# Gadersd/stable-diffusion-xl-burn

Hardware: AMD Instinct MI355X
Metric: images/sec SDXL-base 1024x1024 30-step CFG7.5 (whole job); UNet step ms p50 (higher is better)
Workload: dtype f16; 1 GPU; SDXL-base 1024x1024, n_steps=30 (31 CFG UNet step pairs), CFG 7.5, batch 1 prompt/GPU + VAE decode to u8 (BASELINE configs[1]); precision=f16, vae_dtype=f32_split, weights=synthetic seeded (random-init SDXL-base architecture), mix_classes=0, parallelism=replica x1, 1 prompt per GPU, weights broadcast once over RCCL, hipgraph=True, split_cfg=False, fused_xattn=True, pipelined_decode=False, prompts_per_call=1, full=False, library=stable-diffusion-xl-burn_amd/lib/libsdxl_mi355.so, debug_set=

## Files before the change

stable-diffusion-xl-burn_amd/build.py:

```python
from __future__ import annotations

import hashlib
import os
import subprocess
import sys
from concurrent.futures import ThreadPoolExecutor

HERE = os.path.dirname(os.path.abspath(__file__))
CSRC = os.path.join(HERE, "csrc")
OBJ = os.path.join(HERE, "build")
LIBDIR = os.path.join(HERE, "lib")
LIB = os.path.join(LIBDIR, "libsdxl_mi355.so")
ARCH = "gfx950"
SOURCES = ["igemm.hip", "igemm_glds.hip", "igemm_wreg.hip", "igemm_measure.hip", "norm.hip", "attention.hip", "elementwise.hip", "capi.hip", "capi_ops.hip",
           "select.cpp", "specs.cpp", "weights.cpp", "unet.cpp", "vae.cpp", "sampler.cpp", "clip.cpp", "comm.cpp"]
FLAGS = ["-O3", "-std=c++17", "-fPIC", f"--offload-arch={ARCH}", "-Wall", "-Wno-unused-function",
         "-Wno-unused-result"]


def _hipcc() -> str:
    for c in (os.environ.get("HIPCC"), "/opt/rocm/bin/hipcc", "hipcc"):
        if c and (os.path.isabs(c) and os.path.exists(c) or not os.path.isabs(c)):
            return c
    raise RuntimeError("hipcc not found")


def _measure() -> bool:
    return os.environ.get("SDXL_MEASURE") == "1"

# ... 57 lines not shown
```

stable-diffusion-xl-burn_amd/csrc/capi.hip:

```cpp
#include "capi_internal.h"
#include "select_debug.h"
#include <algorithm>
#include <cstring>

using namespace sdxl;

thread_local std::string sdxl::g_err;

namespace {
template <class H, class F> void create_handle(sdxl_ctx* ctx, H** out, F make) {
  std::unique_ptr<H> h(new H());
  h->ctx = ctx;
  make(*h);
  *out = h.release();
}
UNetCfg to_cfg(const sdxl_unet_config* c) {
  SDXL_REQUIRE(c != nullptr, "null config");
  SDXL_REQUIRE(c->n_levels >= 1 && c->n_levels <= 8, "n_levels out of range");
  UNetCfg u;
  u.adm_in_channels = c->adm_in_channels; u.in_channels = c->in_channels; u.out_channels = c->out_channels;
  u.model_channels = c->model_channels; u.n_head_channels = c->n_head_channels; u.context_dim = c->context_dim;
  u.is_refiner = c->is_refiner != 0;
  for (int i = 0; i < c->n_levels; ++i) { u.channel_mults.push_back(c->channel_mults[i]); u.transformer_depths.push_back(c->transformer_depths[i]); }
  SDXL_REQUIRE(u.model_channels > 0 && u.n_head_channels > 0 && u.context_dim > 0 && u.adm_in_channels > 0, "bad UNet config");
// ... 101 lines not shown
  igemm_glds_init();
  *out = c;
  API_END
}
int sdxl_debug_set(const char* key, int value) {
  API_BEGIN
  SDXL_REQUIRE(key != nullptr, "null key");
  if (select_knob_set(key, value)) return SDXL_OK;
  else if (std::strcmp(key, "igemm_epilogue_staged") == 0) igemm_set_epilogue_staged(value);
  else if (std::strcmp(key, "hl_weights_exact") == 0) igemm_set_hl_weights_exact(value);
  else if (std::strcmp(key, "igemm_warm") == 0) igemm_set_warm(value);
  else if (std::strcmp(key, "splitk_wt") == 0) igemm_set_splitk_wt(value);
  else if (std::strcmp(key, "hl_demote") == 0) unet_set_hl_demote(value);
  else if (std::strcmp(key, "mix_classes") == 0) unet_set_mix_classes(value);
  else if (std::strcmp(key, "wreg_xcd2d") == 0) igemm_set_wreg_xcd2d(value);
#ifdef SDXL_MEASURE
  else if (std::strcmp(key, "xa_vec64") == 0) igemm_set_xa_vec64(value);
  else if (std::strcmp(key, "no_cfg") == 0) g_debug_no_cfg = value != 0;
#endif
  else throw Error(std::string("unknown debug key ") + key);
  API_END
}
int sdxl_debug_warm_schedule(int n, const unsigned* bytes, const unsigned char* host, int* warmed_by) {
  API_BEGIN
  WarmSeq ws;
  for (int j = 0; j < n; ++j)
    ws.seq.push_back(WarmSeq::Item{reinterpret_cast<const void*>((uintptr_t)(j + 1) << 12), bytes[j], host[j] != 0, host[j] ? 14u << 20 : 0u, {nullptr, nullptr, nullptr}, {0u, 0u, 0u}});
  ws.finish();
  for (int j = 0; j < n; ++j) warmed_by[j] = -1;
  for (int i = 0; i < n; ++i)
// ... 569 lines not shown
```

stable-diffusion-xl-burn_amd/csrc/elementwise.hip:

```cpp
#include "kernels.h"
#include <algorithm>
#include <stdexcept>

namespace sdxl {

typedef _Float16 half_t;
typedef _Float16 half8 __attribute__((ext_vector_type(8)));
typedef float f32x4 __attribute__((ext_vector_type(4)));

__device__ __forceinline__ float ld_f(const void* p, size_t i, int dt) {
  if (dt == DT_HL) { const half_t* b = reinterpret_cast<const half_t*>(p) + ((i >> 4) << 5) + (i & 15); return (float)b[0] + (float)b[16]; }
  return dt == DT_F16 ? (float)reinterpret_cast<const half_t*>(p)[i] : reinterpret_cast<const float*>(p)[i];
}
__device__ __forceinline__ void st_f(void* p, size_t i, int dt, float v) {
  if (dt == DT_HL) {
    half_t* b = reinterpret_cast<half_t*>(p) + ((i >> 4) << 5) + (i & 15);
    const half_t hi = (half_t)v;
    b[0] = hi; b[16] = (half_t)(v - (float)hi);
  } else if (dt == DT_F16) reinterpret_cast<half_t*>(p)[i] = (half_t)v; else reinterpret_cast<float*>(p)[i] = v;
}
__device__ __forceinline__ float silu_f(float x) { return x / (1.0f + expf(-x)); }

template <typename WT>
__global__ __launch_bounds__(256) void gemv_kernel(const GemvParams p, int cols) {
// ... 39 lines not shown
            const f32x4 xv = *reinterpret_cast<const f32x4*>(xr + j);
            acc[b] += xv[0] * wv[j] + xv[1] * wv[j + 1] + xv[2] * wv[j + 2] + xv[3] * wv[j + 3];
          }
        }
      }
    }
#pragma unroll
    for (int b = 0; b < 8; ++b) {
#pragma unroll
      for (int o = 32; o > 0; o >>= 1) acc[b] += __shfl_xor(acc[b], o);
    }
    if (lane == 0) {
      for (int b = 0; b < p.Bm; ++b) {
        float v = acc[b] + (p.bias ? p.bias[n] : 0.f);
        if (p.silu_out) v = silu_f(v);
        if (p.Yadd) v += p.Yadd[(size_t)b * p.ldy + n];
        p.Y[(size_t)b * p.ldy + n] = v;
      }
    }
  }
}
void launch_gemv(const GemvParams& pin, hipStream_t s) {
  const int ce = pin.w_dt == DT_F16 ? 8 : 4;
  const int Kx = (pin.K + 64 * ce - 1) / (64 * ce) * (64 * ce);
  const size_t row_bytes = (size_t)Kx * sizeof(float);
  if (row_bytes > 64 * 1024) throw std::runtime_error("gemv: K does not fit the 64 KiB input staging buffer");
  const int rows_per_launch = (int)std::min<size_t>(8, (64 * 1024) / row_bytes);
  for (int b0 = 0; b0 < pin.Bm; b0 += rows_per_launch) {
    GemvParams p = pin;
    p.Bm = std::min(rows_per_launch, pin.Bm - b0);
    p.X = pin.X + (size_t)b0 * pin.ldx;
    p.Y = pin.Y + (size_t)b0 * pin.ldy;
    if (pin.Yadd) p.Yadd = pin.Yadd + (size_t)b0 * pin.ldy;
    const size_t lds = (size_t)p.Bm * row_bytes;
    const int cols = p.N >= 8192 ? 4 : 1;
    dim3 g((p.N + 4 * cols - 1) / (4 * cols));
    if (p.w_dt == DT_F16) hipLaunchKernelGGL(gemv_kernel<half_t>, g, dim3(256), lds, s, p, cols);
    else hipLaunchKernelGGL(gemv_kernel<float>, g, dim3(256), lds, s, p, cols);
  }
}

__global__ __launch_bounds__(256) void softmax_rows_kernel(const float* S, int lds_, void* P, int p_dt, int ldp, int n,
                                                           int npad, float scale, const float* mask, int ldmask,
                                                           int mask_rows, float p_scale, float* p_scale_out) {
  __shared__ float red[8];
  const int row = blockIdx.x, tid = threadIdx.x;
  const float* s = S + (size_t)row * lds_;
  const float* mk = mask ? mask + (size_t)(row % mask_rows) * ldmask : nullptr;
// ... 428 lines not shown
  float z[4];
  seeded_normal4(seeds.v[b], (uint32_t)hw, draw, z);
#pragma unroll
  for (int c = 0; c < 4; ++c) out[((size_t)b * 4 + c) * HW + hw] = z[c];
}
void launch_seeded_noise(float* out, const uint64_t* seeds, uint32_t draw, int n, int HW, hipStream_t s) {
  for (int b0 = 0; b0 < n; b0 += kMaxSeeds) {
    const int nb = std::min(kMaxSeeds, n - b0);
    DdimSeeds k{};
    for (int b = 0; b < nb; ++b) k.v[b] = seeds[b0 + b];
    const size_t total = (size_t)nb * HW;
    hipLaunchKernelGGL(seeded_noise_kernel, dim3((total + 255) / 256), dim3(256), 0, s, out + (size_t)b0 * 4 * HW, k, draw, nb, HW);
  }
}

template <bool SEEDED>
__global__ void ddim_kernel(const DdimParams p, int do_update) {
#pragma clang fp contract(off)
  const size_t i = (size_t)blockIdx.x * blockDim.x + threadIdx.x;
  if (i >= (size_t)p.n * p.HW) return;
  const int b = i / p.HW;
  const int hw = i - (size_t)b * p.HW;
  const int idx = *p.step_idx;
  const int next = do_update ? idx + 1 : 0;
  float x[4];
#pragma unroll
  for (int c = 0; c < 4; ++c) x[c] = p.latent[((size_t)b * 4 + c) * p.HW + hw];
  if (do_update) {
    const StepCoef k = p.table[idx];
#pragma unroll
    for (int c = 0; c < 4; ++c) {
      const float ec = ld_f(p.eps, ((size_t)b * p.HW + hw) * p.eps_ld + c, p.eps_dt);
      float e = ec;
      if (p.use_cfg) {
// ... 25 lines not shown
        if constexpr (SEEDED) zn = z[c]; else zn = p.step_noise[(size_t)next * p.n * 4 * p.HW + e];
        x[c] = p.ref[e] * kn.sqrt_a + zn * kn.sqrt_1ma;
      }
    }
  }
#pragma unroll
  for (int c = 0; c < 4; ++c) p.latent[((size_t)b * 4 + c) * p.HW + hw] = x[c];
  for (int r = 0; r < p.in_rep; ++r)
#pragma unroll
    for (int c = 0; c < 4; ++c) st_f(p.unet_in, ((size_t)(r * p.n + b) * p.HW + hw) * p.in_ld + c, p.in_dt, x[c]);
}
template <bool SEEDED>
__global__ void dpmpp2m_kernel(const DdimParams p, int do_update) {
#pragma clang fp contract(off)
  const size_t i = (size_t)blockIdx.x * blockDim.x + threadIdx.x;
  if (i >= (size_t)p.n * p.HW) return;
  const int b = i / p.HW;
  const int hw = i - (size_t)b * p.HW;
  const int idx = *p.step_idx;
  const int next = do_update ? idx + 1 : 0;
  float x[4];
#pragma unroll
  for (int c = 0; c < 4; ++c) x[c] = p.latent[((size_t)b * 4 + c) * p.HW + hw];
  if (do_update) {
    const StepCoef k = p.table[idx];
    float x0p[4] = {0.f, 0.f, 0.f, 0.f};
    if (k.c_1 != 0.f) {
#pragma unroll
      for (int c = 0; c < 4; ++c) x0p[c] = p.hist[((size_t)b * 4 + c) * p.HW + hw];
    }
// ... 223 lines not shown
```

stable-diffusion-xl-burn_amd/csrc/engine.h:

```cpp
#pragma once
#include "kernels.h"

#include <map>
#include <memory>
#include <stdexcept>
#include <string>
#include <utility>
#include <vector>

namespace sdxl {

struct Error : std::runtime_error {
  explicit Error(const std::string& m) : std::runtime_error(m) {}
};
#define SDXL_HIP(x)                                                                                   \
  do {                                                                                                \
    hipError_t e__ = (x);                                                                             \
    if (e__ != hipSuccess) throw ::sdxl::Error(std::string(#x) + " failed: " + hipGetErrorString(e__)); \
  } while (0)
#define SDXL_REQUIRE(cond, msg)                          \
  do {                                                   \
    if (!(cond)) throw ::sdxl::Error(std::string(msg));  \
  } while (0)

// ... 259 lines not shown
void alloc_ln_operands(Exec& ex, const StPlan& pl, size_t M, int C, const Act& ln, LnOperands& o);
void want_ln_shadow(LnOperands& o, Epi& e, bool sh, LinForm f, const NormW& n);
struct LnIn { const Lin* w; Act a; const float* stat; };
LnIn ln_input(Exec& ex, LnOperands& o, const Lin& plain, const Lin& sh, LinForm f, const NormW& n, const Act& t, int cls);
constexpr size_t kGegluDirectRows = 256;
inline bool geglu_widened(LinForm f, const LnIn& in, size_t M) { return M < kGegluDirectRows && (in.stat || reads_f16(f)); }
struct BlockW { BlockDesc d; ResBlockW res; STW st; Lin conv; };

class UNet {
 public:
  UNet(const UNetCfg& cfg, int compute_dt, int stream_dt, WeightSource& src, hipStream_t st, int mix = 0);
  ~UNet();
  const UNetCfg& cfg() const { return cfg_; }
  void set_context(const float* context, int n_ctx, const float* label, int B, hipStream_t s);
  void forward(int B, int H, int W, const float* t_dev, int t_stride, hipStream_t s);
  void forward_nchw(const float* x, const int* timesteps, const float* context, int n_ctx, const float* label,
                    int B, int H, int W, float* out, hipStream_t s);
  void* unet_in(int B, int H, int W);
  float* eps_out() { return eps_; }
  int compute_dt() const { return cdt_; }
  int mix_classes() const { return mix_; }
  int input_dt() const { return cdt_ == DT_HL ? DT_F32 : cdt_; }
  int attn_dt() const { return cdt_ == DT_HL ? DT_F32 : cdt_; }
  void set_use_graph(bool g) { use_graph_ = g; }
  void set_split_cfg(bool on, int release_offset) { split_cfg_ = on; split_offset_ = release_offset; }
  void set_fused_cross_attention(bool on) { fuse_xattn_ = on; }
  void set_gn_from_producer(bool on) { gn_from_producer_ = on; }
  void profile(int B, int H, int W, float ms[Profiler::NCLS], int launches[Profiler::NCLS], double flops[Profiler::NCLS],
               hipStream_t s);
  float eager_ms(int B, int H, int W, hipStream_t s);
// ... 12 lines not shown
  int mix_ = 0;
  bool mix_knob_ = false;
  bool attn16_ = false;
  DeviceArena warena_;
  std::vector<BlockW> inp_, out_;
  BlockW mid_res1_, mid_res2_;
  Lin lin1_t_, lin2_t_, lin1_l_, lin2_l_, embcat_;
  NormW norm_out_; Lin conv_out_;
  int emb_total_ = 0;
  struct KV { void* k = nullptr; void* vt = nullptr; void* xa = nullptr; void* xa_lo = nullptr; };
  std::vector<std::vector<KV>> kv_;
  std::vector<const STW*> st_list_;
  DeviceArena ctx_arena_;
  int ctx_B_ = 0, n_ctx_ = 0, vt_ld_ctx_ = 0;
  float* label_emb_ = nullptr;
  int pB_ = 0, pH_ = 0, pW_ = 0;
  DeviceArena act_;
  void* in_ = nullptr; float* eps_ = nullptr;
  float *temb_ = nullptr, *g1_ = nullptr, *emb_ = nullptr, *ebias_ = nullptr, *gn_partial_ = nullptr, *tconv_ = nullptr;
  float* skws_[2] = {nullptr, nullptr}; unsigned* skcnt_[2] = {nullptr, nullptr}; size_t skws_bytes_ = 0;
  bool fuse_ln_ = false;
  bool use_graph_ = true;
  bool split_cfg_ = false; int split_offset_ = 0;
  bool plan_split_ = false; int graph_off_ = 0;
  bool fuse_xattn_ = true, plan_xattn_ = true;
  WarmSeq warm_;
  float* attn_xws_[2] = {nullptr, nullptr}; unsigned* attn_xcnt_[2] = {nullptr, nullptr};
  bool graph_warm_ = false;
  size_t attn_xcnt_bytes_ = 0;
  int demote_mask_ = 0, graph_demote_ = 0;
// ... 100 lines not shown
  void sample_latent_inpaint(const Conditioning& c, double cfg_scale, int n_steps, const float* reference,
                             const unsigned char* mask, const float* noise0, const float* step_noise, float* out,
                             hipStream_t s);
  void refine_latent(const float* latent, const Conditioning& c, double cfg_scale, int step_start, int n_steps,
                     const float* noise, float* out, hipStream_t s);
  void sample_latent_seeded(const Conditioning& c, double cfg_scale, int n_steps, const uint64_t* seeds, double eta, float* out,
                            hipStream_t s);
  void sample_latent_inpaint_seeded(const Conditioning& c, double cfg_scale, int n_steps, const float* reference,
                                    const unsigned char* mask, const uint64_t* seeds, double eta, float* out, hipStream_t s);
  void refine_latent_seeded(const float* latent, const Conditioning& c, double cfg_scale, int step_start, int n_steps,
                            const uint64_t* seeds, double eta, float* out, hipStream_t s);
  static std::vector<int> step_schedule(int n_steps, int step_start, int n_train);
  static void solver_coefficients(const double* alphas, int n_train, int n_steps, int step_start, int solver, double eta, double* out);
  void set_solver(int solver);
  int solver() const { return solver_; }
  std::vector<float> step_ms;
  bool time_steps = false;
  float* trace = nullptr; int trace_cap = 0;

 private:
  void ensure_state(size_t elems);
  void diffuse(float* latent, const Conditioning& c, int step_start, int n_steps, double cfg_scale, const float* reference,
               const unsigned char* mask, const float* step_noise, hipStream_t s, const uint64_t* seeds = nullptr, double eta = 0.0);
  std::unique_ptr<UNet> unet_;
  std::vector<double> alphas_;
  int n_train_;
  bool is_refiner_;
  float* latent_ = nullptr; size_t latent_cap_ = 0;
  float* noise_ = nullptr; size_t noise_cap_ = 0;
  float* hist_ = nullptr; size_t hist_cap_ = 0;
// ... 10 lines not shown
```

stable-diffusion-xl-burn_amd/csrc/kernels.h:

```cpp
#pragma once
#include <hip/hip_runtime.h>
#include <stdint.h>
#include <stdexcept>

namespace sdxl {

enum DType : int { DT_F32 = 0, DT_F16 = 1, DT_HL = 2 };

static inline size_t dt_size(int dt) { return dt == DT_F16 ? 2 : 4; }

struct IgemmParams {
  const void* A;
  const void* W;
  const void* Wf;
  int a_dt;
  int B, Hin, Win, Cin, lda;
  int Hout, Wout;
  int ksize, stride, pad, up;
  int M, N, K, Kpad;
  const float* bias;
  const float* ebias;
  int ebias_ld;
  int rpb;
  int act;
// ... 46 lines not shown
  int grid, block, lds;
};
IgemmChoice igemm_select(const IgemmParams& p, int compute_dt, const SelectKnobs& k);
bool igemm_gn_part_ok(const IgemmParams& p, const SelectKnobs& k);
bool igemm_wreg_selected(const IgemmParams& p, const SelectKnobs& k);
bool igemm_wreg_xattn_selected(const IgemmParams& p, const SelectKnobs& k);
bool igemm_xattn_ok(int a_dt, int c_dt, int M, int N, int K, int rpb, int n_ctx);
size_t xattn_pack_bytes(int B, int C);
void launch_xattn_pack(const void* K, const void* Vt, void* out, int B, int C, int n_ctx, int vt_ld, hipStream_t s);
int igemm_splitk_slices(const IgemmParams& p);
size_t igemm_splitk_ws_bytes(int batch, int rows_per_entry, int n_max);
constexpr int kSplitkCounters = 4096;
SelectKnobs igemm_launch_knobs();
void launch_igemm(const IgemmParams& p, int compute_dt, const SelectKnobs& knobs, hipStream_t s);
void launch_igemm(const IgemmParams& p, int compute_dt, hipStream_t s);
void launch_repack_wfrag(const void* w, void* wf, int Npad, int Kpad, hipStream_t s);
void igemm_set_warm(int v);
int igemm_warm_enabled();
void igemm_set_splitk_wt(int v);
void igemm_set_wreg_xcd2d(int v);
void igemm_set_hl_weights_exact(int v);
void igemm_set_xa_vec64(int v);
void igemm_set_epilogue_staged(int v);
#ifdef SDXL_MEASURE
void igemm_set_timeline(void* device_buf);
void igemm_set_wreg_timeline(void* device_buf);
void igemm_set_wide_timeline(void* device_buf);
int igemm_timeline_words();
#endif
constexpr int kMaxDevices = 64;
// ... 71 lines not shown
void attention_set_timeline(void* device_buf);
#endif

void launch_softmax_rows(const float* S, int lds, void* P, int p_dt, int ldp, int rows, int n, int npad, float scale,
                         const float* mask, int ldmask, int mask_rows, hipStream_t s, float p_scale = 1.0f, float* p_scale_out = nullptr);

struct GemvParams {
  const float* X; int ldx;
  const void* W; int w_dt; int Kpad;
  const float* bias;
  float* Y; int ldy;
  const float* Yadd;
  int Bm, N, K;
  int silu_in;
  int silu_out;
};
void launch_gemv(const GemvParams& p, hipStream_t s);

void launch_timestep_embedding(const float* t_dev, int t_stride, float* out, int Bm, int dim, hipStream_t s);
void launch_nchw_to_nhwc(const float* src, int src_batch_stride, void* dst, int dt, int B, int C, int HW, int ldd,
                         float scale, hipStream_t s);
void launch_nhwc_to_nchw(const void* src, int dt, int lds, float* dst, int B, int C, int HW, float scale, hipStream_t s);
void launch_copy_rows(const void* src, int sdt, int lds, void* dst, int ddt, int ldd, int rows, int C, hipStream_t s);
void launch_fill_zero(void* p, size_t bytes, hipStream_t s);
void launch_f16_exact(const float* src, size_t n, float wscale, float* exact, hipStream_t s, bool accumulate = false);
void launch_f32_to_hl(const void* src, int lds, void* dst, int ldd, size_t rows, int C, hipStream_t s);
void launch_f32_to_hl_scaled(const void* src, int lds, void* dst, int ldd, size_t rows, int C, float* scale_io, hipStream_t s, int nb = 1,
                             bool have_partials = false);
unsigned count_nonfinite(const void* src, int dt, int lds, size_t rows, int C, hipStream_t s);
void launch_f16_to_hl(const void* src, int lds, void* dst, int ldd, size_t rows, int C, hipStream_t s);
// ... 22 lines not shown
constexpr uint32_t kDrawInitial = 0;
constexpr uint32_t draw_blend(uint32_t i) { return 1u + 2u * i; }
constexpr uint32_t draw_sigma(uint32_t i) { return 2u + 2u * i; }
constexpr int kMaxSeeds = 8;
struct DdimSeeds { uint64_t v[kMaxSeeds]; };
struct DdimParams {
  float* latent;
  const void* eps; int eps_dt; int eps_ld;
  const StepCoef* table; int* step_idx;
  int n, HW; int use_cfg;
  const float* ref; const unsigned char* mask; const float* step_noise; int n_steps_total;
  int seeded; DdimSeeds seeds;
  void* unet_in; int in_dt; int in_ld; int in_rep;
  float* t_out;
  int solver; float* hist;
};
void launch_ddim_step(const DdimParams& p, int do_update, hipStream_t s);
void launch_seeded_noise(float* out, const uint64_t* seeds, uint32_t draw, int n, int HW, hipStream_t s);
void launch_axpby(float* dst, const float* a, float sa, const float* b, float sb, size_t n, hipStream_t s);
void launch_to_u8_image(const void* src, int dt, int lds, unsigned char* dst, size_t pixels, hipStream_t s);
void launch_from_u8_image(const unsigned char* src, void* dst, int dt, int ldd, size_t pixels, hipStream_t s);

void launch_synth_fill(float* dst, size_t numel, uint64_t key, float scale, float mean, hipStream_t s);
void launch_pack_linear(const float* src, void* dst, int dt, int K, int N, int Kpad, int Npad, int geglu,
                        int n_offset, hipStream_t s, const float* kscale = nullptr,
                        float wscale = 1.0f);
void launch_pack_linear_hilo(const float* src, void* dst, int K, int N, int Npad, int geglu, float lo_scale, hipStream_t s, int mode = 0, int n_offset = 0);
void launch_colsum_packed(const void* wp, int dt, int Kpad, int nrows, float* cs, hipStream_t s, const float* kscale = nullptr, int K = 0, int interleave = 0);
void launch_beta_dot(const float* w, const float* beta, const float* bias, float* out, int K, int N, hipStream_t s);
void launch_pack_conv(const float* src, void* dst, int dt, int Cout, int Cin, int ks, int Kpad, int Npad,
// ... 6 lines not shown
```

stable-diffusion-xl-burn_amd/csrc/sampler.cpp:

```cpp
#include "engine.h"

#include <algorithm>
#include <cmath>

namespace sdxl {

std::vector<int> Diffuser::step_schedule(int n_steps, int step_start, int n_train) {
  SDXL_REQUIRE(n_steps >= 1 && n_steps <= n_train, "n_steps out of range");
  const int step = n_train / n_steps;
  std::vector<int> ts;
  for (int t = n_train - step_start - 1; t >= 0; t -= step) ts.push_back(t);
  return ts;
}

Diffuser::Diffuser(const UNetCfg& cfg, int compute_dt, int stream_dt, WeightSource& src, const float* alphas_host,
                   int n_train, hipStream_t st, int mix)
    : n_train_(n_train), is_refiner_(cfg.is_refiner) {
  unet_.reset(new UNet(cfg, compute_dt, stream_dt, src, st, mix));
  alphas_.resize(n_train);
  for (int i = 0; i < n_train; ++i) alphas_[i] = (double)alphas_host[i];
  SDXL_HIP(hipMalloc((void**)&step_idx_, sizeof(int)));
  SDXL_HIP(hipMalloc((void**)&t_dev_, 8 * sizeof(float)));
}
Diffuser::~Diffuser() {
// ... 41 lines not shown
    const double A = -std::expm1(-(1.0 + eta) * h);
    c[0] = (sigma_p / sigma) * std::exp(-eta * h);
    c[3] = sigma_p * std::sqrt(-std::expm1(-2.0 * eta * h));
    if (have_prev) {
      const double r = h_prev / h;
      c[1] = alpha_p * A * (1.0 + 1.0 / (2.0 * r));
      c[2] = -alpha_p * A / (2.0 * r);
    } else {
      c[1] = alpha_p * A;
      c[2] = 0.0;
    }
    h_prev = h;
    have_prev = true;
  }
}

#ifdef SDXL_MEASURE
bool g_debug_no_cfg = false;
#else
static constexpr bool g_debug_no_cfg = false;
#endif

void Diffuser::diffuse(float* latent, const Conditioning& c, int step_start, int n_steps, double cfg_scale,
                       const float* reference, const unsigned char* mask, const float* step_noise, hipStream_t s,
                       const uint64_t* seeds, double eta) {
  UNet& u = *unet_;
  const UNetCfg& uc = u.cfg();
  const bool single = is_refiner_ || g_debug_no_cfg;
  const int n = c.n, B = single ? n : 2 * n;
  SDXL_REQUIRE(n >= 1 && B <= 8, "batch out of range");
// ... 51 lines not shown
      double sqrt_ap, sqrt_1map, sigma;
      ddim_terms(a, ap, eta, sqrt_ap, sqrt_1map, sigma);
      k.sqrt_ap = (float)sqrt_ap;
      k.sqrt_1map = (float)sqrt_1map;
      k.sigma = (float)sigma;
    }
    tab[i] = k;
  }
  tab[iters] = StepCoef{};
  if (iters + 1 > table_cap_) {
    if (table_) SDXL_HIP(hipFree(table_));
    SDXL_HIP(hipMalloc((void**)&table_, (size_t)(iters + 1) * sizeof(StepCoef)));
    table_cap_ = iters + 1;
  }
  SDXL_HIP(hipMemcpyAsync(table_, tab.data(), (size_t)(iters + 1) * sizeof(StepCoef), hipMemcpyHostToDevice, s));
  SDXL_HIP(hipStreamSynchronize(s));

  DdimParams p{};
  p.latent = latent;
  p.eps = u.eps_out(); p.eps_dt = DT_F32; p.eps_ld = uc.out_channels;
  p.table = table_; p.step_idx = step_idx_;
  p.n = n; p.HW = HW; p.use_cfg = single ? 0 : 1;
  p.ref = reference; p.mask = mask; p.step_noise = step_noise; p.n_steps_total = iters;
  p.unet_in = unet_in; p.in_dt = u.input_dt(); p.in_ld = uc.in_channels; p.in_rep = single ? 1 : 2;
  p.t_out = t_dev_;
  p.solver = solver_; p.hist = hist_;
  if (seeds) {
    p.seeded = 1;
    for (int b = 0; b < n; ++b) p.seeds.v[b] = seeds[b];
  }
  launch_ddim_step(p, 0, s);

  std::vector<hipEvent_t> ev;
  if (time_steps) {
    ev.resize(iters + 1);
    for (auto& e : ev) SDXL_HIP(hipEventCreate(&e));
    SDXL_HIP(hipEventRecord(ev[0], s));
  }
  for (int i = 0; i < iters; ++i) {
    u.forward(B, h, w, t_dev_, 0, s);
    launch_ddim_step(p, 1, s);
    if (trace && i < trace_cap)
      SDXL_HIP(hipMemcpyAsync(trace + (size_t)i * n * 4 * HW, latent, (size_t)n * 4 * HW * sizeof(float), hipMemcpyDeviceToDevice, s));
    if (time_steps) SDXL_HIP(hipEventRecord(ev[i + 1], s));
  }
  if (time_steps) {
    SDXL_HIP(hipEventSynchronize(ev[iters]));
    step_ms.assign(iters, 0.f);
    for (int i = 0; i < iters; ++i) SDXL_HIP(hipEventElapsedTime(&step_ms[i], ev[i], ev[i + 1]));
    for (auto& e : ev) (void)hipEventDestroy(e);
  }
}

static void ensure_latent(float*& buf, size_t& cap, size_t elems) {
  if (elems > cap) {
// ... 82 lines not shown
```

stable-diffusion-xl-burn_amd/csrc/unet.cpp:

```cpp
#include "engine.h"

#include <atomic>
#include <cmath>
#include <cstring>

namespace sdxl {

namespace {
ResBlockW load_res(WeightBuilder& wb, const std::string& p, int cin, int cout, std::vector<std::string>& emb_names,
                   int& emb_off) {
  ResBlockW r;
  r.cin = cin; r.cout = cout;
  r.norm_in = wb.norm(p + ".norm_in");
  r.conv_in = wb.conv(p + ".conv_in");
  r.norm_out = wb.norm(p + ".norm_out");
  r.conv_out = wb.conv(p + ".conv_out");
  r.has_skip = wb.has(p + ".skip_connection.weight");
  if (r.has_skip) r.skip = wb.conv(p + ".skip_connection");
  r.emb_off = emb_off;
  emb_names.push_back(p + ".lin_embed");
  emb_off += cout;
  return r;
}
const std::vector<std::string> kQkv = {".attn1.query", ".attn1.key", ".attn1.value"};
// ... 73 lines not shown
    t.qkv = pack_proj(wb, plan.qkv, qkv, false, plan.qkv_sh ? &t.qkv_sh : nullptr, q + ".norm1");
    t.out1 = pack_proj(wb, plan.out1, {q + kOut1}, false);
    t.n2 = wb.norm(q + ".norm2");
    t.q2 = pack_proj(wb, plan.q2, {q + kQ2}, false, plan.q2_sh ? &t.q2_sh : nullptr, q + ".norm2");
    t.kv2 = wb.fused_linear({q + ".attn2.key", q + ".attn2.value"});
    t.out2 = pack_proj(wb, plan.out2, {q + kOut2}, false);
    t.n3 = wb.norm(q + ".norm3");
    t.geglu = pack_proj(wb, plan.geglu, {q + kGeglu}, true, plan.geglu_sh ? &t.geglu_sh : nullptr, q + ".norm3");
    t.ff = pack_proj(wb, plan.ff, {q + kFf}, false);
    s.blocks.push_back(t);
  }
  s.proj_out = wb.linear(p + ".proj_out");
  return s;
}
void gemv(Exec& ex, const Lin& w, const float* x, int ldx, float* y, int ldy, int Bm, bool silu_in, bool silu_out,
          const float* yadd = nullptr) {
  if (ex.dry) return;
  GemvParams p{};
  p.X = x; p.ldx = ldx; p.W = w.w; p.w_dt = w.dt >= 0 ? w.dt : ex.cdt; p.Kpad = w.Kpad; p.bias = w.b;
  p.Y = y; p.ldy = ldy; p.Yadd = yadd; p.Bm = Bm; p.N = w.N; p.K = w.K;
  p.silu_in = silu_in; p.silu_out = silu_out;
  if (ex.prof) ex.prof->begin(Profiler::OTHER, 2.0 * Bm * (double)w.N * w.K, ex.s);
  launch_gemv(p, ex.s);
  if (ex.prof) ex.prof->end(ex.s);
}
void attention(Exec& ex, const Act& q, const Act& k, const void* vt, int vt_ld, const Act& o, int B, int H, int Nq,
               int Nk, int tag = 0) {
  if (ex.dry) return;
  AttnParams p{};
  p.Q = q.p; p.ldq = q.ld; p.K = k.p; p.ldk = k.ld; p.Vt = vt; p.vt_ld = vt_ld; p.O = o.p; p.ldo = o.ld;
  p.dt = q.dt; p.B = B; p.H = H; p.Nq = Nq; p.Nk = Nk; p.scale = 0.125f; p.mask = nullptr; p.ldmask = 0;
  if (Nq == Nk) { p.xws = ex.attn_xws; p.xcnt = ex.attn_xcnt; }
  if (ex.prof) ex.prof->begin(Profiler::ATTENTION, 4.0 * B * H * (double)Nq * Nk * 64, ex.s, Nq, Nk, B * H, 0, tag ? tag : (Nq == Nk ? DM_ATTN : DM_XATTN));
  launch_attention_d64(p, ex.s);
  {
    const hipError_t le = hipGetLastError();
// ... 95 lines not shown

UNet::UNet(const UNetCfg& cfg, int compute_dt, int stream_dt, WeightSource& src, hipStream_t st, int mix)
    : cfg_(cfg), cdt_(compute_dt), sdt_(stream_dt), mix_(compute_dt == DT_HL ? (mix && g_mix_classes.load() >= 0 ? g_mix_classes.load() : mix) : 0),
      mix_knob_(compute_dt == DT_HL && mix && g_mix_classes.load() >= 0) {
  SDXL_REQUIRE(cfg.n_head_channels == 64, "this engine's fused attention kernel is specialised for 64 channels per head");
  SDXL_REQUIRE(!((compute_dt == DT_F32 || compute_dt == DT_HL) && stream_dt != DT_F32), "f32 / split-operand compute implies an f32 residual stream");
  SDXL_REQUIRE(cfg.model_channels % 32 == 0, "GroupNorm(32) needs model_channels % 32 == 0");
  fuse_ln_ = compute_dt == DT_F16 && stream_dt == DT_F16;
  build_weights(src, st);
}
UNet::~UNet() {
  if (graph_) (void)hipGraphExecDestroy(graph_);
  if (ev_fork_) (void)hipEventDestroy(ev_fork_);
  if (ev_join_) (void)hipEventDestroy(ev_join_);
  if (s2_) (void)hipStreamDestroy(s2_);
}

void UNet::build_weights(WeightSource& src, hipStream_t st) {
  const std::vector<ParamSpec> specs = unet_param_specs(cfg_);
  std::vector<BlockDesc> inp, out; BlockDesc mid;
  unet_block_plan(cfg_, inp, mid, out);
  std::vector<std::pair<std::string, int>> sts;
  auto has_st = [](const BlockDesc& d) { return d.kind == BK_REST || d.kind == BK_RESTU; };
  for (size_t i = 0; i < inp.size(); ++i) if (has_st(inp[i])) sts.push_back({"input_blocks." + std::to_string(i) + ".transformer", inp[i].depth});
  sts.push_back({"middle_block.transformer", mid.depth});
  for (size_t i = 0; i < out.size(); ++i) if (has_st(out[i])) sts.push_back({"output_blocks." + std::to_string(i) + ".transformer", out[i].depth});
  std::vector<StPlan> plans;
  std::vector<std::string> f16_names;
  auto plan_all = [&]() {
    plans.clear(); f16_names.clear();
// ... 326 lines not shown
  ex.act->reset(mk);
}

void UNet::run(Exec& ex, const float* t_dev, int t_stride, int b0, int nb) {
  const int B = nb, H = pH_, W = pW_;
  const int mc = cfg_.model_channels, emb = 4 * mc;
  float* temb = temb_ + (size_t)b0 * mc;
  float* g1 = g1_ + (size_t)b0 * emb;
  float* embv = emb_ + (size_t)b0 * emb;
  float* ebias = ebias_ + (size_t)b0 * emb_total_;
  const float* label_emb = label_emb_ ? label_emb_ + (size_t)b0 * emb : nullptr;
  void* in = (char*)in_ + (size_t)b0 * H * W * cfg_.in_channels * dt_size(input_dt());
  float* eps = eps_ + (size_t)b0 * H * W * cfg_.out_channels;
  ex.ebias = ebias; ex.b0 = b0;
  ex.gn_partial = gn_partial_ + (size_t)b0 * groupnorm_workspace_floats(1, 32);
  if (!ex.dry) launch_timestep_embedding(t_dev + (size_t)b0 * t_stride, t_stride, temb, B, mc, ex.s);
  gemv(ex, lin1_t_, temb, mc, g1, emb, B, false, true);
  gemv(ex, lin2_t_, g1, emb, embv, emb, B, false, false, label_emb);
  gemv(ex, embcat_, embv, emb, ebias, emb_total_, B, true, false);

  const int n_in = (int)inp_.size(), n_out = (int)out_.size();
  SDXL_REQUIRE(n_in == n_out, "input/output block count mismatch");
  std::vector<int> hs_h(n_in), hs_w(n_in), hs_c(n_in);
  {
    int h = H, w = W;
    for (int i = 0; i < n_in; ++i) {
      const BlockDesc& d = inp_[i].d;
      if (d.kind == BK_DOWN) { h = (h - 1) / 2 + 1; w = (w - 1) / 2 + 1; }
      hs_h[i] = h; hs_w[i] = w; hs_c[i] = d.c_out;
    }
  }
  std::vector<Act> cat(n_out);
  std::vector<int> cx(n_out);
  for (int j = 0; j < n_out; ++j) {
// ... 148 lines not shown
  plan_xattn_ = fuse_xattn_;
  plan_gn_ = gn_from_producer_;
  if (!had_kv) kv_.clear();
  act_.reset(m);
  const size_t peak = act_.peak;
  act_.dry = false;
  act_.reserve(peak + 4096);
  act_.off = 0; act_.peak = 0;
  persist();
  for (int c = 0; c < 2; ++c) if (skcnt_[c]) SDXL_HIP(hipMemset(skcnt_[c], 0, kSplitkCounters * sizeof(unsigned)));
  for (int c = 0; c < (split ? 2 : 1); ++c) if (attn_xcnt_[c] && attn16_) SDXL_HIP(hipMemset(attn_xcnt_[c], 0, attn_xcnt_bytes_));
}

void* UNet::unet_in(int B, int H, int W) { ensure_plan(B, H, W); return in_; }

void UNet::forward(int B, int H, int W, const float* t_dev, int t_stride, hipStream_t s) {
  ensure_plan(B, H, W);
  SDXL_REQUIRE(ctx_B_ == B && !kv_.empty(), "set_context must be called with the same batch before forward");
  Exec ex; ex.s = s; ex.cdt = cdt_; ex.sdt = sdt_; ex.act = &act_; ex.gn_partial = gn_partial_; ex.demote = demote_mask_;
  ex.splitk_ws = skws_[0]; ex.splitk_ws_bytes = skws_bytes_; ex.splitk_cnt = skcnt_[0];
  if (attn16_) { ex.attn_xws = attn_xws_[0]; ex.attn_xcnt = attn_xcnt_[0]; }
  const bool warming = cdt_ == DT_F16 && !plan_split_ && igemm_warm_enabled();
  if (warming) { ex.warm = &warm_; if (!warm_.ready) { warm_.seq.clear(); warm_.recording = true; } }
  const size_t m = act_.mark();
  auto go = [&]() {
    warm_.pos = 0;
    if (!plan_split_) { run(ex, t_dev, t_stride, 0, B); if (warm_.recording) warm_.finish(); return; }
    Exec e2; e2.s = s2_; e2.cdt = cdt_; e2.sdt = sdt_; e2.act = &act2_; e2.demote = demote_mask_;
    e2.splitk_ws = skws_[1]; e2.splitk_ws_bytes = skws_bytes_; e2.splitk_cnt = skcnt_[1];
    if (attn16_) { e2.attn_xws = attn_xws_[1]; e2.attn_xcnt = attn_xcnt_[1]; }
// ... 93 lines not shown
```

stable-diffusion-xl-burn_amd/csrc/weights.cpp:

```cpp
#include "engine.h"

#include <cstdio>
#include <cstdlib>
#include <cstring>
#include <cmath>

namespace sdxl {

DeviceArena::~DeviceArena() { if (base) (void)hipFree(base); }
void DeviceArena::reserve(size_t bytes) {
  if (bytes <= cap && base) return;
  if (base) { SDXL_HIP(hipFree(base)); base = nullptr; }
  SDXL_HIP(hipMalloc((void**)&base, bytes));
  cap = bytes;
}
void* DeviceArena::alloc(size_t bytes) {
  const size_t a = round_up(off, 256);
  off = a + bytes;
  if (off > peak) peak = off;
  if (dry) return (void*)(uintptr_t)(a + 256);
  if (off > cap) throw Error("device arena overflow (" + std::to_string(off) + " > " + std::to_string(cap) + ")");
  return base + a;
}

// ... 449 lines not shown
      auto ext = [&](const void* q, size_t sz) { const char* c = reinterpret_cast<const char*>(q); if (q && c >= hi && c - hi <= (64 << 10)) hi = c + sz; };
      ext(w.b, (size_t)w.Npad * 4); ext(w.cs, (size_t)w.Npad * 4); ext(w.ln_eps, 4);
    }
    if (ws.recording) {
      if (p.xa_k) ws.seq.push_back(WarmSeq::Item{p.xa_k, (unsigned)xattn_pack_bytes(p.M / p.rpb, p.N), false, 0u, {nullptr, nullptr, nullptr}, {0u, 0u, 0u}});
      const unsigned budget = host ? 14u << 20 : 0u;
      ws.seq.push_back(WarmSeq::Item{lo, (unsigned)(hi - lo), host, budget, {nullptr, nullptr, nullptr}, {0u, 0u, 0u}});
    } else if (ws.ready) {
      if (p.xa_k) ++ws.pos;
      if (ws.pos < ws.seq.size()) {
        const WarmSeq::Item& it = ws.seq[ws.pos++];
        if (it.w == lo) for (int r = 0; r < 3; ++r) { p.warm[r] = it.warm[r]; p.warm_bytes[r] = it.warm_bytes[r]; }
      }
    }
  }
  launch_igemm(p, w.dt >= 0 ? w.dt : ex.cdt, knobs, ex.s);
  {
    const hipError_t le = hipGetLastError();
    if (le != hipSuccess)
      throw Error(std::string("implicit-GEMM launch failed (") + hipGetErrorString(le) + "): M=" + std::to_string(p.M) + " N=" + std::to_string(p.N) +
                  " K=" + std::to_string(p.K) + " ksize=" + std::to_string(p.ksize) + " a_dt=" + std::to_string(p.a_dt) + " c_dt=" + std::to_string(p.c_dt) +
                  " compute=" + std::to_string(w.dt >= 0 ? w.dt : ex.cdt) + " act=" + std::to_string(p.act) + " n_split=" + std::to_string(p.n_split));
  }
  if (ex.prof) ex.prof->end(ex.s);
  {
    static const bool nan_check = std::getenv("SDXL_NAN_CHECK") != nullptr;
    hipStreamCaptureStatus cs = hipStreamCaptureStatusNone;
    if (nan_check && hipStreamIsCapturing(ex.s, &cs) == hipSuccess && cs == hipStreamCaptureStatusNone) {
      const int nout = p.act == 1 ? p.N / 2 : (p.n_split < p.N ? p.n_split : p.N);
      const unsigned bo = nout > 0 ? count_nonfinite(out.p, out.dt, out.ld, (size_t)p.M, nout, ex.s) : 0;
      if (bo) {
// ... 64 lines not shown
```

Measured before the change: 1.444 images/sec.

## Add skinny 3x3 conv kernel and precompute timestep embeddings per run

```diff
diff --git a/stable-diffusion-xl-burn_amd/build.py b/stable-diffusion-xl-burn_amd/build.py
--- a/stable-diffusion-xl-burn_amd/build.py
+++ b/stable-diffusion-xl-burn_amd/build.py
@@ -12,7 +12,7 @@
 LIBDIR = os.path.join(HERE, "lib")
 LIB = os.path.join(LIBDIR, "libsdxl_mi355.so")
 ARCH = "gfx950"
-SOURCES = ["igemm.hip", "igemm_glds.hip", "igemm_wreg.hip", "igemm_measure.hip", "norm.hip", "attention.hip", "elementwise.hip", "capi.hip", "capi_ops.hip",
+SOURCES = ["igemm.hip", "igemm_glds.hip", "igemm_wreg.hip", "igemm_narrow.hip", "igemm_measure.hip", "norm.hip", "attention.hip", "elementwise.hip", "capi.hip", "capi_ops.hip",
            "select.cpp", "specs.cpp", "weights.cpp", "unet.cpp", "vae.cpp", "sampler.cpp", "clip.cpp", "comm.cpp"]
 FLAGS = ["-O3", "-std=c++17", "-fPIC", f"--offload-arch={ARCH}", "-Wall", "-Wno-unused-function",
          "-Wno-unused-result"]
diff --git a/stable-diffusion-xl-burn_amd/csrc/capi.hip b/stable-diffusion-xl-burn_amd/csrc/capi.hip
--- a/stable-diffusion-xl-burn_amd/csrc/capi.hip
+++ b/stable-diffusion-xl-burn_amd/csrc/capi.hip
@@ -139,6 +139,8 @@
   else if (std::strcmp(key, "hl_demote") == 0) unet_set_hl_demote(value);
   else if (std::strcmp(key, "mix_classes") == 0) unet_set_mix_classes(value);
   else if (std::strcmp(key, "wreg_xcd2d") == 0) igemm_set_wreg_xcd2d(value);
+  else if (std::strcmp(key, "conv_narrow") == 0) conv_narrow_set(value);
+  else if (std::strcmp(key, "temb_in_step") == 0) Diffuser::set_temb_in_step(value != 0);
 #ifdef SDXL_MEASURE
   else if (std::strcmp(key, "xa_vec64") == 0) igemm_set_xa_vec64(value);
   else if (std::strcmp(key, "no_cfg") == 0) g_debug_no_cfg = value != 0;
diff --git a/stable-diffusion-xl-burn_amd/csrc/elementwise.hip b/stable-diffusion-xl-burn_amd/csrc/elementwise.hip
--- a/stable-diffusion-xl-burn_amd/csrc/elementwise.hip
+++ b/stable-diffusion-xl-burn_amd/csrc/elementwise.hip
@@ -77,7 +77,7 @@
       for (int b = 0; b < p.Bm; ++b) {
         float v = acc[b] + (p.bias ? p.bias[n] : 0.f);
         if (p.silu_out) v = silu_f(v);
-        if (p.Yadd) v += p.Yadd[(size_t)b * p.ldy + n];
+        if (p.Yadd) v += p.Yadd[(p.yadd_bcast ? (size_t)0 : (size_t)b * p.ldy) + n];
         p.Y[(size_t)b * p.ldy + n] = v;
       }
     }
@@ -94,7 +94,7 @@
     p.Bm = std::min(rows_per_launch, pin.Bm - b0);
     p.X = pin.X + (size_t)b0 * pin.ldx;
     p.Y = pin.Y + (size_t)b0 * pin.ldy;
-    if (pin.Yadd) p.Yadd = pin.Yadd + (size_t)b0 * pin.ldy;
+    if (pin.Yadd && !pin.yadd_bcast) p.Yadd = pin.Yadd + (size_t)b0 * pin.ldy;
     const size_t lds = (size_t)p.Bm * row_bytes;
     const int cols = p.N >= 8192 ? 4 : 1;
     dim3 g((p.N + 4 * cols - 1) / (4 * cols));
@@ -553,10 +553,17 @@
   }
 }
 
+__device__ __forceinline__ void copy_ebias_row(const DdimParams& p, int next) {
+  if (!p.eb_table || next >= p.n_steps_total) return;
+  const float* src = p.eb_table + (size_t)next * p.eb_row;
+  const int nthreads = gridDim.x * blockDim.x;
+  for (int j = blockIdx.x * blockDim.x + threadIdx.x; j < p.eb_row; j += nthreads) p.eb_dst[j] = src[j];
+}
 template <bool SEEDED>
 __global__ void ddim_kernel(const DdimParams p, int do_update) {
 #pragma clang fp contract(off)
   const size_t i = (size_t)blockIdx.x * blockDim.x + threadIdx.x;
+  copy_ebias_row(p, do_update ? *p.step_idx + 1 : 0);
   if (i >= (size_t)p.n * p.HW) return;
   const int b = i / p.HW;
   const int hw = i - (size_t)b * p.HW;
@@ -612,6 +619,7 @@
 __global__ void dpmpp2m_kernel(const DdimParams p, int do_update) {
 #pragma clang fp contract(off)
   const size_t i = (size_t)blockIdx.x * blockDim.x + threadIdx.x;
+  copy_ebias_row(p, do_update ? *p.step_idx + 1 : 0);
   if (i >= (size_t)p.n * p.HW) return;
   const int b = i / p.HW;
   const int hw = i - (size_t)b * p.HW;
diff --git a/stable-diffusion-xl-burn_amd/csrc/engine.h b/stable-diffusion-xl-burn_amd/csrc/engine.h
--- a/stable-diffusion-xl-burn_amd/csrc/engine.h
+++ b/stable-diffusion-xl-burn_amd/csrc/engine.h
@@ -297,6 +297,9 @@
   const UNetCfg& cfg() const { return cfg_; }
   void set_context(const float* context, int n_ctx, const float* label, int B, hipStream_t s);
   void forward(int B, int H, int W, const float* t_dev, int t_stride, hipStream_t s);
+  const float* embed_timesteps(const float* t_dev, int t_stride, int n_t, int B, hipStream_t s);
+  float* ebias_buf(int B, int H, int W) { ensure_plan(B, H, W); return ebias_; }
+  int emb_total() const { return emb_total_; }
   void forward_nchw(const float* x, const int* timesteps, const float* context, int n_ctx, const float* label,
                     int B, int H, int W, float* out, hipStream_t s);
   void* unet_in(int B, int H, int W);
@@ -339,6 +342,7 @@
   DeviceArena ctx_arena_;
   int ctx_B_ = 0, n_ctx_ = 0, vt_ld_ctx_ = 0;
   float* label_emb_ = nullptr;
+  float* tt_buf_ = nullptr; size_t tt_cap_ = 0;
   int pB_ = 0, pH_ = 0, pW_ = 0;
   DeviceArena act_;
   void* in_ = nullptr; float* eps_ = nullptr;
@@ -469,6 +473,7 @@
   static void solver_coefficients(const double* alphas, int n_train, int n_steps, int step_start, int solver, double eta, double* out);
   void set_solver(int solver);
   int solver() const { return solver_; }
+  static void set_temb_in_step(bool on);
   std::vector<float> step_ms;
   bool time_steps = false;
   float* trace = nullptr; int trace_cap = 0;
diff --git a/stable-diffusion-xl-burn_amd/csrc/igemm_narrow.hip b/stable-diffusion-xl-burn_amd/csrc/igemm_narrow.hip
--- /dev/null
+++ b/stable-diffusion-xl-burn_amd/csrc/igemm_narrow.hip
@@ -0,0 +1,170 @@
+#include "kernels.h"
+#include <algorithm>
+#include <atomic>
+
+namespace sdxl {
+
+typedef _Float16 half_t;
+typedef _Float16 half8 __attribute__((ext_vector_type(8)));
+typedef float f32x4 __attribute__((ext_vector_type(4)));
+
+struct NarrowParams {
+  const void* A; const void* W; const float* bias; void* C;
+  const float* acc_scale; const float* a_scale; int a_scale_rpb;
+  int B, H, Wd, Cin, lda, N, Kpad, ldc, c_dt, nstore;
+  int vec;
+};
+
+constexpr int kSkinnyRpw = 2;
+template <bool KSPLIT>
+__global__ __launch_bounds__(256) void conv3x3_skinny_kernel(const NarrowParams p) {
+  extern __shared__ __attribute__((aligned(16))) unsigned char smem[];
+  constexpr int ESZ = 4;
+  constexpr int CB = 64;
+  constexpr int U = KSPLIT ? 2 : 4;
+  constexpr int FR = 4;
+  constexpr int FW = 8;
+  constexpr int RPW = KSPLIT ? 1 : kSkinnyRpw;
+  const int tid = threadIdx.x, lane = tid & 63, wave = tid >> 6;
+  const int j = lane & 15, q = lane >> 4;
+  const int rowb = p.Kpad * ESZ + (KSPLIT ? 0 : 16);
+  if constexpr (!KSPLIT) {
+    const int vec_per_row = p.Kpad * ESZ / 16;
+    for (int i = tid; i < p.N * vec_per_row; i += 256) {
+      const int n = i / vec_per_row, v = i - n * vec_per_row;
+      *reinterpret_cast<f32x4*>(smem + (size_t)n * rowb + v * 16) =
+          *reinterpret_cast<const f32x4*>(reinterpret_cast<const unsigned char*>(p.W) + (size_t)n * p.Kpad * ESZ + v * 16);
+    }
+    __syncthreads();
+  }
+  const int nrow = j < p.N ? j : p.N - 1;
+  const unsigned char* wrow;
+  if constexpr (KSPLIT) wrow = reinterpret_cast<const unsigned char*>(p.W) + (size_t)nrow * rowb;
+  else wrow = smem + (size_t)nrow * rowb;
+  const int wq = (q & 1) * 16;
+  const int b = blockIdx.z;
+  const int x = blockIdx.x * 16 + j;
+  const int cpb = p.Cin / CB, T = 9 * cpb;
+  const int ks_begin = KSPLIT ? wave * T / 4 : 0, ks_end = KSPLIT ? (wave + 1) * T / 4 : T;
+  const unsigned char* A = reinterpret_cast<const unsigned char*>(p.A);
+  const size_t rowbytes = (size_t)p.lda * ESZ;
+  half8 zero8;
+#pragma unroll
+  for (int e = 0; e < 8; ++e) zero8[e] = (half_t)0.f;
+  for (int rep = 0; rep < RPW; ++rep) {
+    const int y = KSPLIT ? (int)blockIdx.y : ((int)blockIdx.y * RPW + rep) * 4 + wave;
+    const bool rowok = y < p.H;
+    f32x4 acc = {0.f, 0.f, 0.f, 0.f};
+    int tap = ks_begin / cpb, cb = ks_begin - tap * cpb;
+    for (int ks0 = ks_begin; ks0 < ks_end; ks0 += U) {
+      half8 fa[U][FR];
+      half8 fw[KSPLIT ? U : 1][FW];
+      unsigned koff[U];
+#pragma unroll
+      for (int u = 0; u < U; ++u) {
+        const bool live = ks0 + u < ks_end;
+        const int ky = (tap * 11) >> 5, kx = tap - ky * 3;
+        const int yy = y + ky - 1, xx = x + kx - 1;
+        const bool ok = live && rowok && yy >= 0 && yy < p.H && xx >= 0 && xx < p.Wd;
+        const unsigned char* src = A + (((size_t)b * p.H + yy) * p.Wd + xx) * rowbytes + (size_t)cb * CB * ESZ + q * 16;
+#pragma unroll
+        for (int f = 0; f < FR; ++f) fa[u][f] = ok ? *reinterpret_cast<const half8*>(src + f * 64) : zero8;
+        koff[u] = live ? (unsigned)(((size_t)tap * p.Cin + (size_t)cb * CB) * ESZ) : 0u;
+        if constexpr (KSPLIT) {
+#pragma unroll
+          for (int f = 0; f < 4; ++f) {
+            fw[u][2 * f] = live ? *reinterpret_cast<const half8*>(wrow + koff[u] + f * 64 + wq) : zero8;
+            fw[u][2 * f + 1] = live ? *reinterpret_cast<const half8*>(wrow + koff[u] + f * 64 + 32 + wq) : zero8;
+          }
+        }
+        if (live && ++cb == cpb) { cb = 0; ++tap; }
+      }
+#pragma unroll
+      for (int u = 0; u < U; ++u) {
+        if (ks0 + u >= ks_end) continue;
+#pragma unroll
+        for (int f = 0; f < 4; ++f) {
+          half8 w1, w2;
+          if constexpr (KSPLIT) { w1 = fw[u][2 * f]; w2 = fw[u][2 * f + 1]; }
+          else {
+            w1 = *reinterpret_cast<const half8*>(wrow + koff[u] + f * 64 + wq);
+            w2 = *reinterpret_cast<const half8*>(wrow + koff[u] + f * 64 + 32 + wq);
+          }
+          if (q >= 2) w2 = zero8;
+          acc = __builtin_amdgcn_mfma_f32_16x16x32_f16(w1, fa[u][f], acc, 0, 0, 0);
+          acc = __builtin_amdgcn_mfma_f32_16x16x32_f16(w2, fa[u][f], acc, 0, 0, 0);
+        }
+      }
+    }
+    if constexpr (KSPLIT) {
+      f32x4* red = reinterpret_cast<f32x4*>(smem);
+      red[wave * 64 + lane] = acc;
+      __syncthreads();
+      if (wave != 0) continue;
+      acc = red[lane];
+#pragma unroll
+      for (int w = 1; w < 4; ++w) { const f32x4 o = red[w * 64 + lane]; acc[0] += o[0]; acc[1] += o[1]; acc[2] += o[2]; acc[3] += o[3]; }
+    }
+    if (!rowok || x >= p.Wd) continue;
+    const int n0 = 4 * q;
+    if (n0 >= p.nstore) continue;
+    const size_t m = ((size_t)b * p.H + y) * p.Wd + x;
+    float sc = p.acc_scale ? p.acc_scale[0] : 1.f;
+    if (p.a_scale) sc *= p.a_scale[p.a_scale_rpb > 0 ? m / (size_t)p.a_scale_rpb : 0];
+    float v[4];
+#pragma unroll
+    for (int r = 0; r < 4; ++r) v[r] = acc[r] * sc + ((p.bias && n0 + r < p.N) ? p.bias[n0 + r] : 0.f);
+    if (p.c_dt == DT_F32 && p.vec && n0 + 4 <= p.nstore) {
+      *reinterpret_cast<f32x4*>(reinterpret_cast<float*>(p.C) + m * p.ldc + n0) = f32x4{v[0], v[1], v[2], v[3]};
+    } else {
+#pragma unroll
+      for (int r = 0; r < 4; ++r)
+        if (n0 + r < p.nstore) {
+          if (p.c_dt == DT_F16) reinterpret_cast<half_t*>(p.C)[m * p.ldc + n0 + r] = (half_t)v[r];
+          else reinterpret_cast<float*>(p.C)[m * p.ldc + n0 + r] = v[r];
+        }
+    }
+  }
+}
+
+static std::atomic<int> g_conv_narrow{1};
+void conv_narrow_set(int v) { g_conv_narrow = v; }
+
+constexpr int kSkinnyRowsPixels = 1 << 17;
+
+static bool skinny_ksplit(const IgemmParams& p) { return (long long)p.Hin * p.Win < kSkinnyRowsPixels; }
+static int skinny_lds(const IgemmParams& p) {
+  if (skinny_ksplit(p)) return 4 * 64 * 16;
+  return p.N * (p.Kpad * 4 + 16);
+}
+
+int conv_narrow_takes(const IgemmParams& p, int compute_dt) {
+  if (!g_conv_narrow.load()) return 0;
+  if (p.ksize != 3 || p.stride != 1 || p.pad != 1 || p.up || p.Hout != p.Hin || p.Wout != p.Win || p.M <= 0) return 0;
+  if (p.K != 9 * p.Cin || p.N < 1 || p.N > 16) return 0;
+  if (p.ebias || p.act != 0 || p.R || p.ln_stat || p.stat_out || p.gn_part || p.xa_k || p.shadow || p.Ct || p.n_split < 1) return 0;
+  if (p.c_dt != DT_F16 && p.c_dt != DT_F32) return 0;
+  if (compute_dt != DT_HL || p.a_dt != DT_HL || p.Cin % 64 != 0) return 0;
+  if (p.lda % 8 != 0 || (reinterpret_cast<uintptr_t>(p.A) & 15) != 0 || (reinterpret_cast<uintptr_t>(p.W) & 15) != 0) return 0;
+  if (p.B > 65535 || p.Hin > 65535) return 0;
+  return skinny_lds(p) <= 64 * 1024 ? 2 : 0;
+}
+
+bool launch_conv_narrow(const IgemmParams& p, int compute_dt, hipStream_t s) {
+  if (!conv_narrow_takes(p, compute_dt)) return false;
+  NarrowParams q{};
+  q.A = p.A; q.W = p.W; q.bias = p.bias; q.C = p.C;
+  q.acc_scale = p.acc_scale; q.a_scale = p.a_scale; q.a_scale_rpb = p.a_scale_rpb;
+  q.B = p.B; q.H = p.Hin; q.Wd = p.Win; q.Cin = p.Cin; q.lda = p.lda; q.N = p.N; q.Kpad = p.Kpad; q.ldc = p.ldc; q.c_dt = p.c_dt;
+  q.nstore = p.n_split < p.N ? p.n_split : p.N;
+  const size_t cbytes = p.c_dt == DT_F16 ? 2 : 4;
+  q.vec = ((reinterpret_cast<uintptr_t>(p.C) & 15) == 0 && ((size_t)p.ldc * cbytes) % 16 == 0) ? 1 : 0;
+  const bool ksplit = skinny_ksplit(p);
+  const int lds = skinny_lds(p);
+  const dim3 grid((p.Win + 15) / 16, ksplit ? p.Hin : (p.Hin + 4 * kSkinnyRpw - 1) / (4 * kSkinnyRpw), p.B);
+  if (ksplit) hipLaunchKernelGGL(conv3x3_skinny_kernel<true>, grid, dim3(256), lds, s, q);
+  else hipLaunchKernelGGL(conv3x3_skinny_kernel<false>, grid, dim3(256), lds, s, q);
+  return true;
+}
+
+}
diff --git a/stable-diffusion-xl-burn_amd/csrc/kernels.h b/stable-diffusion-xl-burn_amd/csrc/kernels.h
--- a/stable-diffusion-xl-burn_amd/csrc/kernels.h
+++ b/stable-diffusion-xl-burn_amd/csrc/kernels.h
@@ -84,6 +84,9 @@
 SelectKnobs igemm_launch_knobs();
 void launch_igemm(const IgemmParams& p, int compute_dt, const SelectKnobs& knobs, hipStream_t s);
 void launch_igemm(const IgemmParams& p, int compute_dt, hipStream_t s);
+int conv_narrow_takes(const IgemmParams& p, int compute_dt);
+bool launch_conv_narrow(const IgemmParams& p, int compute_dt, hipStream_t s);
+void conv_narrow_set(int v);
 void launch_repack_wfrag(const void* w, void* wf, int Npad, int Kpad, hipStream_t s);
 void igemm_set_warm(int v);
 int igemm_warm_enabled();
@@ -185,6 +188,7 @@
   int Bm, N, K;
   int silu_in;
   int silu_out;
+  int yadd_bcast;
 };
 void launch_gemv(const GemvParams& p, hipStream_t s);
 
@@ -237,6 +241,7 @@
   void* unet_in; int in_dt; int in_ld; int in_rep;
   float* t_out;
   int solver; float* hist;
+  const float* eb_table; float* eb_dst; int eb_row;
 };
 void launch_ddim_step(const DdimParams& p, int do_update, hipStream_t s);
 void launch_seeded_noise(float* out, const uint64_t* seeds, uint32_t draw, int n, int HW, hipStream_t s);
diff --git a/stable-diffusion-xl-burn_amd/csrc/sampler.cpp b/stable-diffusion-xl-burn_amd/csrc/sampler.cpp
--- a/stable-diffusion-xl-burn_amd/csrc/sampler.cpp
+++ b/stable-diffusion-xl-burn_amd/csrc/sampler.cpp
@@ -1,7 +1,9 @@
 #include "engine.h"
 
 #include <algorithm>
+#include <atomic>
 #include <cmath>
+#include <cstddef>
 
 namespace sdxl {
 
@@ -79,6 +81,9 @@
     have_prev = true;
   }
 }
+
+static std::atomic<bool> g_temb_in_step{false};
+void Diffuser::set_temb_in_step(bool on) { g_temb_in_step = on; }
 
 #ifdef SDXL_MEASURE
 bool g_debug_no_cfg = false;
@@ -160,6 +165,10 @@
     table_cap_ = iters + 1;
   }
   SDXL_HIP(hipMemcpyAsync(table_, tab.data(), (size_t)(iters + 1) * sizeof(StepCoef), hipMemcpyHostToDevice, s));
+  const bool temb_table = !g_temb_in_step;
+  const float* eb_table = nullptr;
+  static_assert(sizeof(StepCoef) % sizeof(float) == 0 && offsetof(StepCoef, t) == 0, "the table's t column is read as strided floats");
+  if (temb_table) eb_table = u.embed_timesteps(reinterpret_cast<const float*>(table_), (int)(sizeof(StepCoef) / sizeof(float)), iters, B, s);
   SDXL_HIP(hipStreamSynchronize(s));
 
   DdimParams p{};
@@ -171,6 +180,7 @@
   p.unet_in = unet_in; p.in_dt = u.input_dt(); p.in_ld = uc.in_channels; p.in_rep = single ? 1 : 2;
   p.t_out = t_dev_;
   p.solver = solver_; p.hist = hist_;
+  if (temb_table) { p.eb_table = eb_table; p.eb_dst = u.ebias_buf(B, h, w); p.eb_row = B * u.emb_total(); }
   if (seeds) {
     p.seeded = 1;
     for (int b = 0; b < n; ++b) p.seeds.v[b] = seeds[b];
@@ -184,7 +194,7 @@
     SDXL_HIP(hipEventRecord(ev[0], s));
   }
   for (int i = 0; i < iters; ++i) {
-    u.forward(B, h, w, t_dev_, 0, s);
+    u.forward(B, h, w, temb_table ? nullptr : t_dev_, 0, s);
     launch_ddim_step(p, 1, s);
     if (trace && i < trace_cap)
       SDXL_HIP(hipMemcpyAsync(trace + (size_t)i * n * 4 * HW, latent, (size_t)n * 4 * HW * sizeof(float), hipMemcpyDeviceToDevice, s));
diff --git a/stable-diffusion-xl-burn_amd/csrc/unet.cpp b/stable-diffusion-xl-burn_amd/csrc/unet.cpp
--- a/stable-diffusion-xl-burn_amd/csrc/unet.cpp
+++ b/stable-diffusion-xl-burn_amd/csrc/unet.cpp
@@ -111,12 +111,12 @@
   return s;
 }
 void gemv(Exec& ex, const Lin& w, const float* x, int ldx, float* y, int ldy, int Bm, bool silu_in, bool silu_out,
-          const float* yadd = nullptr) {
+          const float* yadd = nullptr, bool yadd_bcast = false) {
   if (ex.dry) return;
   GemvParams p{};
   p.X = x; p.ldx = ldx; p.W = w.w; p.w_dt = w.dt >= 0 ? w.dt : ex.cdt; p.Kpad = w.Kpad; p.bias = w.b;
   p.Y = y; p.ldy = ldy; p.Yadd = yadd; p.Bm = Bm; p.N = w.N; p.K = w.K;
-  p.silu_in = silu_in; p.silu_out = silu_out;
+  p.silu_in = silu_in; p.silu_out = silu_out; p.yadd_bcast = yadd_bcast;
   if (ex.prof) ex.prof->begin(Profiler::OTHER, 2.0 * Bm * (double)w.N * w.K, ex.s);
   launch_gemv(p, ex.s);
   if (ex.prof) ex.prof->end(ex.s);
@@ -242,6 +242,7 @@
   if (ev_fork_) (void)hipEventDestroy(ev_fork_);
   if (ev_join_) (void)hipEventDestroy(ev_join_);
   if (s2_) (void)hipStreamDestroy(s2_);
+  if (tt_buf_) (void)hipFree(tt_buf_);
 }
 
 void UNet::build_weights(WeightSource& src, hipStream_t st) {
@@ -598,10 +599,12 @@
   float* eps = eps_ + (size_t)b0 * H * W * cfg_.out_channels;
   ex.ebias = ebias; ex.b0 = b0;
   ex.gn_partial = gn_partial_ + (size_t)b0 * groupnorm_workspace_floats(1, 32);
-  if (!ex.dry) launch_timestep_embedding(t_dev + (size_t)b0 * t_stride, t_stride, temb, B, mc, ex.s);
-  gemv(ex, lin1_t_, temb, mc, g1, emb, B, false, true);
-  gemv(ex, lin2_t_, g1, emb, embv, emb, B, false, false, label_emb);
-  gemv(ex, embcat_, embv, emb, ebias, emb_total_, B, true, false);
+  if (t_dev) {
+    if (!ex.dry) launch_timestep_embedding(t_dev + (size_t)b0 * t_stride, t_stride, temb, B, mc, ex.s);
+    gemv(ex, lin1_t_, temb, mc, g1, emb, B, false, true);
+    gemv(ex, lin2_t_, g1, emb, embv, emb, B, false, false, label_emb);
+    gemv(ex, embcat_, embv, emb, ebias, emb_total_, B, true, false);
+  }
 
   const int n_in = (int)inp_.size(), n_out = (int)out_.size();
   SDXL_REQUIRE(n_in == n_out, "input/output block count mismatch");
@@ -780,6 +783,33 @@
 
 void* UNet::unet_in(int B, int H, int W) { ensure_plan(B, H, W); return in_; }
 
+const float* UNet::embed_timesteps(const float* t_dev, int t_stride, int n_t, int B, hipStream_t s) {
+  SDXL_REQUIRE(ctx_B_ == B && label_emb_, "set_context must be called with the same batch before embed_timesteps");
+  SDXL_REQUIRE(n_t >= 1, "no timesteps");
+  const int mc = cfg_.model_channels, emb = 4 * mc;
+  const size_t n_temb = (size_t)n_t * mc, n_g1 = (size_t)n_t * emb, n_embv = (size_t)B * n_t * emb, n_tab = (size_t)n_t * B * emb_total_;
+  const size_t need = n_temb + n_g1 + n_embv + n_tab;
+  if (need > tt_cap_) {
+    if (tt_buf_) SDXL_HIP(hipFree(tt_buf_));
+    tt_buf_ = nullptr; tt_cap_ = 0;
+    SDXL_HIP(hipMalloc((void**)&tt_buf_, need * sizeof(float)));
+    tt_cap_ = need;
+  }
+  float* tab = tt_buf_;
+  float* temb = tab + n_tab;
+  float* g1 = temb + n_temb;
+  float* embv = g1 + n_g1;
+  Exec ex; ex.s = s; ex.cdt = cdt_; ex.sdt = sdt_;
+  launch_timestep_embedding(t_dev, t_stride, temb, n_t, mc, s);
+  gemv(ex, lin1_t_, temb, mc, g1, emb, n_t, false, true);
+  for (int b = 0; b < B; ++b) {
+    float* eb = embv + (size_t)b * n_t * emb;
+    gemv(ex, lin2_t_, g1, emb, eb, emb, n_t, false, false, label_emb_ + (size_t)b * emb, true);
+    gemv(ex, embcat_, eb, emb, tab + (size_t)b * emb_total_, B * emb_total_, n_t, true, false);
+  }
+  return tab;
+}
+
 void UNet::forward(int B, int H, int W, const float* t_dev, int t_stride, hipStream_t s) {
   ensure_plan(B, H, W);
   SDXL_REQUIRE(ctx_B_ == B && !kv_.empty(), "set_context must be called with the same batch before forward");
diff --git a/stable-diffusion-xl-burn_amd/csrc/weights.cpp b/stable-diffusion-xl-burn_amd/csrc/weights.cpp
--- a/stable-diffusion-xl-burn_amd/csrc/weights.cpp
+++ b/stable-diffusion-xl-burn_amd/csrc/weights.cpp
@@ -487,7 +487,7 @@
       }
     }
   }
-  launch_igemm(p, w.dt >= 0 ? w.dt : ex.cdt, knobs, ex.s);
+  if (knobs.igemm_variant != 0 || !launch_conv_narrow(p, w.dt >= 0 ? w.dt : ex.cdt, ex.s)) launch_igemm(p, w.dt >= 0 ? w.dt : ex.cdt, knobs, ex.s);
   {
     const hipError_t le = hipGetLastError();
     if (le != hipSuccess)
```

Result: no change. 1.448 images/sec (median of 6 runs) (+0.2%).
